# yoshitomo-matsubara/sc2-benchmark

Measured on AMD Instinct MI355X. Metric: images/s + bpp, Entropic-Student ResNet-50 224^2, higher is better.
Workload: dtype bf16

## Files before the change

include/sc2_bottleneck.h:

```cpp
#ifndef SC2_BOTTLENECK_H
#define SC2_BOTTLENECK_H

#include <stddef.h>
#include <stdint.h>

#ifdef __cplusplus
extern "C" {
#endif

#define SC2_OK 0
#define SC2_ERR_INVALID_ARG (-1)
#define SC2_ERR_UNSUPPORTED (-2)
#define SC2_ERR_DOMAIN (-3)
#define SC2_ERR_ZERO_PMF (-4)
#define SC2_ERR_LAUNCH (-5)
#define SC2_ERR_NO_DEVICE (-6)
#define SC2_ERR_INTERNAL (-7)

#define SC2_ABI_VERSION 51
int sc2_abi_version(void);

typedef struct sc2_policy {
    int32_t struct_bytes;
    int32_t conv_patch3;
// ... 81 lines not shown
    int32_t OH, OW;
    int32_t a_op;
    int32_t epilogue;
    int32_t out_format;
    int32_t Kpad;
    int32_t Cout_pad;
    int32_t out_H, out_W, out_stride_h, out_stride_w, out_off_h, out_off_w;
    int32_t k_order;
    int32_t dil_h, dil_w;
} sc2_conv_desc;

int sc2_conv_weight_rows(int Cout);
int sc2_conv_weight_pitch(int K);

int sc2_conv_fused_gdn_supported(const sc2_conv_desc *d);
int sc2_conv_patch_supported(const sc2_conv_desc *d);
int sc2_conv2d_fwd(const sc2_conv_desc *d, const void *x, const void *w_packed, void *y,
                   const void *ep_x, const float *ep_beta, void *stream);

int sc2_gdn1_bwd_gemm(const sc2_conv_desc *d, const void *x, const void *w_packed, void *y, void *y2, const void *ep_x,
                      const void *ep_x2, const float *ep_beta, void *stream);

int sc2_gdn1_rows_supported(int C);
int sc2_gdn1_rows_fwd(const void *x, const void *gamma_frag, const float *beta, void *y, long long M, int C, int inverse,
                      void *stream);
int sc2_gdn1_rows_bwd(const void *x, const void *gy, const void *gamma_frag, const void *gamma_t_frag, const float *beta,
                      void *d_norm, void *dx, float *d_beta, long long M, int C, int inverse, void *stream);
int sc2_colsum_bf16(const void *x, long long M, int C, float *out, void *stream);

int sc2_conv1x1_pair_supported(int K1, int C, int N2);
int sc2_conv1x1_pair_fwd(const void *o, const void *w3_frag, const float *b3, const void *identity, void *h,
                         const void *w1_frag, const float *b1, void *u, long long M, int K1, int C, int N2, void *stream);

int sc2_nchw_f32_to_nhwc_f32(const float *x, float *y, int N, int C, int H, int W, int Cpad, void *stream);
int sc2_conv_f32_chunk_channels(int Cout);
int sc2_conv2d_f32_fwd(const sc2_conv_desc *d, const float *x, const float *w_frag, void *y, const float *ep_x,
                       const float *ep_beta, void *stream);

int sc2_conv2x2_gdn512_supported(int Cin, int Cout, int KH, int KW, int stride, int pad);
int sc2_conv2x2_gdn512_fwd(const void *x, const void *w_packed, int Kpad, const void *gamma_frag, const float *beta,
                           void *y, void *t_out, int N, int H, int W, int Cin, int inverse, void *stream);

int sc2_conv0_gdn96_supported(int Cin_pairs, int Cout, int W_pairs);
int sc2_conv0_gdn96_fwd(const void *x_pairs, const void *w_frag, const void *gamma_frag, const float *beta, void *y, void *t_out,
                        int N, int H, int W_pairs, int inverse, void *stream);
int sc2_conv0_gdn96_nchw_fwd(const float *x_nchw, const void *w_frag, const void *gamma_frag, const float *beta, void *y,
                             int N, int H, int W, int inverse, void *stream);

int sc2_conv1x1_kres_supported(int Cin, int Cout, int stride);
int sc2_conv1x1_kres_fwd(const void *x, const void *w_frag, const float *bias, void *y, int N, int H, int W, int Cin, int Cout,
                         int stride, int relu, void *stream);

int sc2_conv2x2_c48_supported(int H, int W, int Cin, int Cout);
int sc2_conv2x2_c48_fwd(const void *x, const void *w_frag, const float *medians, void *y, int N, int H, int W, int Cin, int Cout,
                        int symbols, void *stream);

int sc2_conv1x1_win_supported(int Cin, int Cout, int stride);
int sc2_conv1x1_win_fwd(const void *x, const void *w_frag, const float *bias, const void *residual, const void *mask, void *y, int N,
                        int H, int W, int Cin, int Cout, int stride, int relu, void *stream);

int sc2_conv3x3_win_supported(int H, int W, int Cin, int Cout);
int sc2_conv3x3_win_fwd(const void *x, const void *w_frag, const float *bias, const void *mask, void *y, int N, int H, int W, int Cin,
                        int Cout, int relu, void *stream);

int sc2_conv3x3s2_win_supported(int H, int W, int Cin, int Cout);
int sc2_conv3x3s2_win_fwd(const void *x, const void *w_frag, const float *bias, void *y, int N, int H, int W, int Cin, int Cout,
// ... 133 lines not shown
```

sc2-benchmark_amd/build.py:

```python
import os
import subprocess
import sys
from concurrent.futures import ThreadPoolExecutor

HERE = os.path.dirname(os.path.abspath(__file__))
CSRC = os.path.join(HERE, 'csrc')
OBJ = os.path.join(CSRC, '_obj')
LIB = os.path.join(HERE, 'libsc2amd.so')
SOURCES = ['conv_inst_e.hip', 'conv_inst_f.hip', 'conv_inst_g.hip', 'conv_inst_h.hip', 'conv_inst_a.hip', 'conv_inst_b.hip',
           'conv_inst_c.hip', 'conv_inst_d.hip', 'conv_dec_persist.hip', 'conv_igemm.hip', 'conv_gdn512.hip', 'gdn512_rows.hip', 'bn.hip', 'gdn96_strips.hip', 'conv0_gdn96.hip', 'conv2_gdn48.hip', 'conv2x2_c48.hip', 'conv1x1_stream.hip', 'conv1x1_pair.hip', 'conv1x1_kres.hip', 'conv3x3_win.hip', 'conv1x1_win.hip', 'conv2x2_win.hip',
           'conv_f32.hip', 'loss.hip', 'conv_wgrad.hip', 'gdn_bwd.hip', 'entropy.hip', 'gaussian.hip', 'ar_context.hip', 'rans.hip', 'layout.hip', 'diag.hip', 'abi.cpp', 'cdf_host.cpp', 'rans_host.cpp']
HEADERS = [os.path.join(CSRC, 'sc2_common.h'), os.path.join(CSRC, 'conv_igemm_impl.h'),
           os.path.join(HERE, '..', 'include', 'sc2_bottleneck.h')]
HIPCC = os.environ.get('HIPCC', '/opt/rocm/bin/hipcc')
FLAGS = ['--offload-arch=gfx950', '-O3', '-fPIC', '-std=c++17', '-Wall', '-Wno-unused-function',
         '-D__HIP_PLATFORM_AMD__=1']


def _stale(target, deps):
    if not os.path.exists(target):
        return True
    t = os.path.getmtime(target)
    return any(os.path.getmtime(d) > t for d in deps)


def _compile(src):
    path = os.path.join(CSRC, src)
    obj = os.path.join(OBJ, src + '.o')
    if _stale(obj, [path] + HEADERS):
        cmd = [HIPCC] + FLAGS + ['-x', 'hip', '-c', path, '-o', obj]
        subprocess.check_call(cmd)
    return obj


def build(force=False, verbose=False):
    os.makedirs(OBJ, exist_ok=True)
    if force:
        for f in os.listdir(OBJ):
            os.remove(os.path.join(OBJ, f))
    with ThreadPoolExecutor(max_workers=min(8, os.cpu_count() or 1)) as ex:
        objs = list(ex.map(_compile, SOURCES))
    if _stale(LIB, objs):
        cmd = [HIPCC, '--offload-arch=gfx950', '-shared', '-fPIC', '-o', LIB] + objs
# ... 9 lines not shown
```

sc2-benchmark_amd/head.py:

```python
import os

import torch
from torch import nn

from . import hip
from .resnet import Bottleneck, FrozenBatchNorm2d


def _fold(conv, bn):
    w = conv.weight.detach().float()
    if bn is None:
        scale = torch.ones(w.shape[0], dtype=torch.float32, device=w.device)
        bias = torch.zeros(w.shape[0], dtype=torch.float32, device=w.device)
    elif isinstance(bn, (nn.BatchNorm2d, FrozenBatchNorm2d)):
        gamma = bn.weight.detach().float() if bn.weight is not None else torch.ones_like(bn.running_mean)
        beta = bn.bias.detach().float() if bn.bias is not None else torch.zeros_like(bn.running_mean)
        scale = gamma * torch.rsqrt(bn.running_var.detach().float() + bn.eps)
        bias = beta - bn.running_mean.detach().float() * scale
    else:
        raise TypeError('cannot fold {}'.format(type(bn)))
    w = w * scale.reshape(-1, 1, 1, 1)
    order = hip.preferred_k_order(w.shape[1], w.shape[2], w.shape[3])
    return hip.pack_conv_weight(w, order), bias.contiguous(), order, w

# ... 86 lines not shown
        if self.w_win1 is not None and epilogue in (hip.EPI_BIAS, hip.EPI_BIAS_RELU, hip.EPI_BIAS_ADD_RELU) and \
                max(x.numel(), x.shape[0] * x.shape[1] * x.shape[2] * self.cout) * 2 < 0x7FF00000:
            return hip.conv1x1_win_fwd(x, self.w_win1, self.b, stride=self.stride[0],
                                       residual=ep_x if epilogue == hip.EPI_BIAS_ADD_RELU else None,
                                       relu=epilogue != hip.EPI_BIAS, tag=self.tag)
        if self.stream and epilogue in (hip.EPI_BIAS, hip.EPI_BIAS_RELU, hip.EPI_BIAS_ADD_RELU):
            return hip.conv1x1_stream_fwd(x, self.w_frag, self.b, stride=self.stride[0],
                                          residual=ep_x if epilogue == hip.EPI_BIAS_ADD_RELU else None,
                                          relu=epilogue != hip.EPI_BIAS, tag=self.tag)
        if self.kres and epilogue in (hip.EPI_BIAS, hip.EPI_BIAS_RELU):
            return hip.conv1x1_kres_fwd(x, self.w_frag, self.b, stride=self.stride[0], relu=epilogue == hip.EPI_BIAS_RELU,
                                        tag=self.tag)
        if self.w_win is not None and epilogue in (hip.EPI_BIAS, hip.EPI_BIAS_RELU) and x.numel() * 2 < 0x7FF00000 and \
                hip.conv3x3_win_supported(x.shape[1], x.shape[2], x.shape[3], self.cout, self.k[0], self.k[1], self.stride, self.pad):
            return hip.conv3x3_win_fwd(x, self.w_win, self.b, relu=epilogue == hip.EPI_BIAS_RELU, tag=self.tag, stride=self.stride[0])
        return hip.conv2d_fwd(x, self.w, self.cout, self.k[0], self.k[1], self.stride, self.pad, epilogue=epilogue,
                              ep_x=ep_x, ep_beta=self.b, tag=self.tag, k_order=self.k_order)


class HipHead(object):

    def __init__(self, layers, fc):
        self.blocks = []
        for li, layer in layers:
            for bi, blk in enumerate(layer):
                if not isinstance(blk, Bottleneck):
                    raise hip.Sc2Error('HipHead supports torchvision Bottleneck blocks, got {}'.format(type(blk)))
                t = 'head.{}.{}'.format(li, bi)
                ds = None
                if blk.downsample is not None:
                    ds = _Conv(blk.downsample[0], blk.downsample[1], t + '.ds')
                self.blocks.append((_Conv(blk.conv1, blk.bn1, t + '.c1'), _Conv(blk.conv2, blk.bn2, t + '.c2'),
                                    _Conv(blk.conv3, blk.bn3, t + '.c3'), ds))
        self.fc = None
        if fc is not None:
            w = fc.weight.detach().float().reshape(fc.out_features, fc.in_features, 1, 1)
            cout_pad = (fc.out_features + 7) // 8 * 8
            if cout_pad != fc.out_features:
                w = torch.cat([w, torch.zeros(cout_pad - fc.out_features, fc.in_features, 1, 1, device=w.device)])
            b = torch.zeros(cout_pad, device=w.device)
            if fc.bias is not None:
                b[:fc.out_features] = fc.bias.detach().float()
            self.fc = (hip.pack_conv_weight(w), b.contiguous(), cout_pad, fc.out_features)
            self.fc_frag = None
            if fc.in_features % 128 == 0 and hip.host_policy.fc_kernel:
                n16 = (fc.out_features + 15) // 16 * 16
                w16 = torch.zeros(n16, fc.in_features, device=w.device)
                w16[:fc.out_features] = fc.weight.detach().float()
                b16 = torch.zeros(n16, device=w.device)
                if fc.bias is not None:
                    b16[:fc.out_features] = fc.bias.detach().float()
                self.fc_frag = (hip.pack_weight_fragments(w16), b16.contiguous())

    @staticmethod
    def _pair_ok(c3, c1n):
        return (c3.k == (1, 1) and c1n.k == (1, 1) and c3.stride == (1, 1) and c1n.stride == (1, 1) and c3.stream and
                c3.w2d is not None and c1n.w2d is not None and c3.w2d.shape[0] == c1n.w2d.shape[1] and
                hip.conv1x1_pair_supported(c3.w2d.shape[1], c3.cout, c1n.cout))

    @staticmethod
    def _pair_w1(c1n):
        if getattr(c1n, 'w_frag_pair', None) is None:
            c1n.w_frag_pair = hip.pack_weight_fragments(c1n.w_folded.reshape(c1n.w_folded.shape[0], c1n.w_folded.shape[1]))
        return c1n.w_frag_pair

    def tail_spec(self):
        c1, _, _, ds = self.blocks[0]
        if ds is None or c1.w2d is None or ds.w2d is None:
            return None
        if tuple(c1.w2d.shape) != (128, 256) or c1.stride != (1, 1) or tuple(ds.w2d.shape) != (512, 256) or ds.stride != (2, 2):
            return None
        return c1.w2d, c1.b, ds.w2d, ds.b

    def _side_stream(self, t):
        if not t.is_cuda or torch.cuda.is_current_stream_capturing():
            return None
        cur = torch.cuda.current_stream(t.device)
        pool = self.__dict__.setdefault('_side_streams', {})
        s = pool.get(cur.cuda_stream)
        if s is None:
            s = pool[cur.cuda_stream] = torch.cuda.Stream(device=t.device)
        return s

    def forward(self, x_nhwc, with_pool=True, pre=None):
        h = x_nhwc
        o_next = None
        side = self._side_stream(h if h is not None else pre[0]) if hip.host_policy.head_ds_side_stream else None
        for bi, (c1, c2, c3, ds) in enumerate(self.blocks):
            join = None
            if bi == 0 and pre is not None:
                o, identity = pre
            else:
                if ds is not None and side is not None:
                    cur = torch.cuda.current_stream(h.device)
                    fork = torch.cuda.Event()
                    fork.record(cur)
                    side.wait_event(fork)
                    h.record_stream(side)
                    with torch.cuda.stream(side):
                        identity = ds(h, hip.EPI_BIAS)
                        join = torch.cuda.Event()
                        join.record(side)
                    identity.record_stream(cur)
                else:
                    identity = h if ds is None else ds(h, hip.EPI_BIAS)
                o = o_next if o_next is not None else c1(h, hip.EPI_BIAS_RELU)
            o_next = None
            o = c2(o, hip.EPI_BIAS_RELU)
            if join is not None:
                torch.cuda.current_stream(h.device).wait_event(join)
            nxt = self.blocks[bi + 1] if bi + 1 < len(self.blocks) else None
            if nxt is not None and self._pair_ok(c3, nxt[0]) and o.numel() // o.shape[-1] * c3.cout * 2 < 0x7FF00000:
                h, o_next = hip.conv1x1_pair_fwd(o, c3.w_frag, c3.b, identity.contiguous(), self._pair_w1(nxt[0]), nxt[0].b,
                                                 tag=c3.tag + '+' + nxt[0].tag)
            else:
                h = c3(o, hip.EPI_BIAS_ADD_RELU, ep_x=identity)
        if not with_pool:
            return h.permute(0, 3, 1, 2)
        if self.fc is None:
            return hip.avgpool_nhwc(h.contiguous(), want_f32=True)[0]
        w, b, cout_pad, n_cls = self.fc
# ... 45 lines not shown
```

sc2-benchmark_amd/hip.py:

```python
import ctypes
import os

import torch

_HERE = os.path.dirname(os.path.abspath(__file__))
LIB_PATH = os.environ.get('SC2_LIB') or os.path.join(_HERE, 'libsc2amd.so')
_lib = None

AOP_NONE, AOP_ABS, AOP_SQUARE = 0, 1, 2
EPI_NONE, EPI_GDN, EPI_IGDN, EPI_BIAS, EPI_BIAS_RELU, EPI_BIAS_ADD_RELU, EPI_FUSED_GDN, EPI_FUSED_IGDN, \
    EPI_BIAS_LEAKY_RELU, EPI_GDN2, EPI_IGDN2 = range(11)
FUSABLE_GDN_CHANNELS = (32, 48, 64, 96)
OUT_BF16_NHWC, OUT_F32_NCHW, OUT_F32_NHWC, OUT_I32_NCHW_SYM = 0, 1, 2, 3
EB_NOISE, EB_DEQUANTIZE = 0, 1
EB_PARAM_STRIDE = 64

ABI_SYMBOLS = [
    'sc2_abi_version', 'sc2_last_error', 'sc2_device_count', 'sc2_policy_default', 'sc2_policy_set', 'sc2_policy_get',
    'sc2_nchw_f32_to_nhwc_bf16', 'sc2_nhwc_bf16_to_nchw_f32', 'sc2_avgpool_nhwc', 'sc2_maxpool_nhwc', 'sc2_bn_ws_floats', 'sc2_bn_train_fwd', 'sc2_bn_train_bwd', 'sc2_fc_fwd',
    'sc2_conv_weight_rows', 'sc2_conv_weight_pitch', 'sc2_conv_fused_gdn_supported', 'sc2_conv_patch_supported',
    'sc2_conv2d_fwd', 'sc2_gdn1_bwd_gemm', 'sc2_colsum_bf16', 'sc2_nchw_f32_to_nhwc_f32', 'sc2_conv_f32_chunk_channels', 'sc2_conv2d_f32_fwd',
    'sc2_conv2x2_gdn512_supported', 'sc2_conv2x2_gdn512_fwd', 'sc2_conv1x1_stream_supported', 'sc2_conv1x1_stream_mask_supported', 'sc2_conv1x1_stream_fwd', 'sc2_conv1x1_pair_supported', 'sc2_conv1x1_pair_fwd',
    'sc2_conv0_gdn96_supported', 'sc2_conv0_gdn96_fwd', 'sc2_conv0_gdn96_nchw_fwd', 'sc2_conv2_gdn48_supported', 'sc2_conv2_gdn48_fwd', 'sc2_conv2x2_c48_supported', 'sc2_conv2x2_c48_fwd', 'sc2_conv1x1_kres_supported', 'sc2_conv1x1_kres_fwd', 'sc2_conv1x1_win_supported', 'sc2_conv1x1_win_fwd', 'sc2_conv3x3_win_supported', 'sc2_conv3x3_win_fwd', 'sc2_conv3x3s2_win_supported', 'sc2_conv3x3s2_win_fwd', 'sc2_conv2x2_win_supported', 'sc2_conv2x2_win_fwd', 'sc2_conv2x2_win_tail_supported', 'sc2_conv2x2_win_tail_fwd', 'sc2_conv2d_wgrad', 'sc2_gdn_bwd_pre', 'sc2_gdn_bwd_post', 'sc2_gdn1_rows_supported', 'sc2_gdn1_rows_fwd', 'sc2_gdn1_rows_bwd',
    'sc2_eb_forward', 'sc2_eb_backward', 'sc2_eb_bits_partial_len', 'sc2_eb_symbols', 'sc2_eb_dequantize',
    'sc2_gc_forward', 'sc2_gc_backward', 'sc2_gc_symbols_indexes', 'sc2_gc_dequantize',
    'sc2_pmf_to_quantized_cdf',
    'sc2_rans_max_bytes', 'sc2_rans_workspace_bytes', 'sc2_rans_encode_batch', 'sc2_rans_decode_batch', 'sc2_rans_decode_dequantize_batch', 'sc2_rans_decode_dequantize_batch_ev',
    'sc2_mse_partial_len', 'sc2_mse_sum_bf16', 'sc2_mse_grad_bf16', 'sc2_relu_bwd_bf16', 'sc2_relu_bwd_mse_bf16',
    'sc2_ar_scan', 'sc2_rans_decode_resume',
    'sc2_rans_host_tables_create', 'sc2_rans_host_tables_destroy', 'sc2_rans_host_rcp_div', 'sc2_rans_code_host', 'sc2_clock_probe', 'sc2_rans_encode_host', 'sc2_rans_decode_host',
]


class ConvDesc(ctypes.Structure):
    _fields_ = [(n, ctypes.c_int32) for n in (
        'N', 'H', 'W', 'Cin', 'Cout', 'KH', 'KW', 'stride_h', 'stride_w', 'pad_h', 'pad_w', 'OH', 'OW',
        'a_op', 'epilogue', 'out_format', 'Kpad', 'Cout_pad', 'out_H', 'out_W', 'out_stride_h', 'out_stride_w',
        'out_off_h', 'out_off_w', 'k_order', 'dil_h', 'dil_w')]


class ArScanArgs(ctypes.Structure):
    _fields_ = ([(n, ctypes.c_int32) for n in ('B', 'H', 'W', 'M', 'C1p', 'C2p', 'n_table', 'n_cdfs', 'cdf_stride', 'pix0',
                                               'pix1', 'decode')] +
                [('scale_bound', ctypes.c_float), ('cdf_entries', ctypes.c_int32), ('stride', ctypes.c_int64)] +
                [(n, ctypes.c_void_p) for n in ('wc', 'bc', 'w1', 'p1', 'w2', 'b2', 'w3', 'b3', 'scale_table', 'y_hat_pad',
                                                'y_hat_nhwc', 'y', 'symbols', 'indexes', 'buf', 'io_offset', 'io_nbytes',
                                                'cdfs', 'cdf_sizes', 'offsets', 'st_x', 'st_pos', 'status',
                                                'gaussian_params')])


class Sc2Error(RuntimeError):
    pass


POLICY_FIELDS = ('struct_bytes', 'conv_patch3', 'conv_s2', 'conv_persist', 'conv_half', 'conv_big4', 'conv_no_big', 'conv_force_big',
                 'conv_no_epx', 'conv_debug', 'conv_chunk', 'w2_run', 'win_half', 'win_dbg', 'win_stamps', 'p1_half',
                 'p1_nbuf', 'pair_alt', 'f32_persist0', 'dec_stagger', 'wgrad_wgs', 'rans_lds_pad_kb', 'rans_pad_waves', 'rans_ragged2',
                 'rans_ragged2_waves', 'rans_lut8', 'rans_dq_lds', 'wgrad_ct')


class Policy(ctypes.Structure):
    _fields_ = [(n, ctypes.c_int32) for n in POLICY_FIELDS] + [('reserved', ctypes.c_int32 * 6)]


class HostPolicy(object):
    conv_patch = True
    k_order_tap = False
    b_tile_major = True
    conv0_fused = True
    conv2_fused = True
    conv_kres = 1
    conv_win = True
    conv_win_s2 = True
    conv2x2_win = True
    w2_tail = True
    conv_stream = True
    conv1x1_pair = True
    conv_c48 = True
    conv1x1_win = '1'
    conv_dilation = True
    fc_kernel = True
    dense_head = True
    rans_fused_dq = True
    gdn_rows = True
    gdn_bwd_fused = True
    dgrad_win_halves = True
    train_fused_conv2 = True
    train_fused_dec0 = True
    train_fused_conv0 = True
    bn_train_hip = True
    conv_train_hip = True
    pack_gather = True
    maxpool_hip = True
    relu_mask_fused = True
    mse_fused = True
    teacher_stream = True
    host_coder_max_streams = 64
    head_ds_side_stream = False
    pipeline_host_steps = True
    eval_graphs = True
    eval_graph_max_batch = 1


host_policy = HostPolicy()


def get_policy():
    p = Policy()
    lib().sc2_policy_get(ctypes.byref(p))
    return p
# ... 68 lines not shown
    L.sc2_conv_weight_rows.argtypes = [i32]
    L.sc2_conv_weight_pitch.argtypes = [i32]
    L.sc2_conv_fused_gdn_supported.argtypes = [ctypes.POINTER(ConvDesc)]
    L.sc2_conv_patch_supported.argtypes = [ctypes.POINTER(ConvDesc)]
    L.sc2_conv2d_fwd.argtypes = [ctypes.POINTER(ConvDesc), vp, vp, vp, vp, vp, vp]
    L.sc2_gdn1_bwd_gemm.argtypes = [ctypes.POINTER(ConvDesc), vp, vp, vp, vp, vp, vp, vp, vp]
    L.sc2_colsum_bf16.argtypes = [vp, ctypes.c_longlong, i32, vp, vp]
    L.sc2_nchw_f32_to_nhwc_f32.argtypes = [vp, vp, i32, i32, i32, i32, i32, vp]
    L.sc2_conv_f32_chunk_channels.argtypes = [i32]
    L.sc2_conv2d_f32_fwd.argtypes = [ctypes.POINTER(ConvDesc), vp, vp, vp, vp, vp, vp]
    L.sc2_conv2x2_gdn512_supported.argtypes = [i32] * 6
    L.sc2_conv2x2_gdn512_fwd.argtypes = [vp, vp, i32, vp, vp, vp, vp, i32, i32, i32, i32, i32, vp]
    L.sc2_conv0_gdn96_supported.argtypes = [i32, i32, i32]
    L.sc2_conv0_gdn96_fwd.argtypes = [vp, vp, vp, vp, vp, vp, i32, i32, i32, i32, vp]
    L.sc2_conv0_gdn96_nchw_fwd.argtypes = [vp, vp, vp, vp, vp, i32, i32, i32, i32, vp]
    L.sc2_conv1x1_kres_supported.argtypes = [i32, i32, i32]
    L.sc2_conv1x1_kres_fwd.argtypes = [vp, vp, vp, vp, i32, i32, i32, i32, i32, i32, i32, vp]
    L.sc2_conv3x3_win_supported.argtypes = [i32, i32, i32, i32]
    L.sc2_conv3x3_win_fwd.argtypes = [vp, vp, vp, vp, vp, i32, i32, i32, i32, i32, i32, vp]
    L.sc2_conv3x3s2_win_supported.argtypes = [i32, i32, i32, i32]
    L.sc2_conv1x1_win_supported.argtypes = [i32, i32, i32]
    L.sc2_conv2x2_c48_supported.argtypes = [i32, i32, i32, i32]
    L.sc2_conv2x2_c48_fwd.argtypes = [vp, vp, vp, vp, i32, i32, i32, i32, i32, i32, vp]
    L.sc2_conv1x1_win_fwd.argtypes = [vp, vp, vp, vp, vp, vp, i32, i32, i32, i32, i32, i32, i32, vp]
    L.sc2_conv3x3s2_win_fwd.argtypes = [vp, vp, vp, vp, i32, i32, i32, i32, i32, i32, vp]
    L.sc2_conv2x2_win_supported.argtypes = [i32, i32, i32, i32, i32]
    L.sc2_conv2x2_win_fwd.argtypes = [vp, vp, vp, vp, i32, i32, i32, i32, i32, i32, i32, i32, i32, vp]
    L.sc2_conv2x2_win_tail_supported.argtypes = [i32, i32, i32]
    L.sc2_conv2x2_win_tail_fwd.argtypes = [vp, vp, vp, vp, vp, vp, vp, i32, i32, i32, i32, vp]
    L.sc2_conv2_gdn48_supported.argtypes = [i32, i32, i32]
    L.sc2_conv2_gdn48_fwd.argtypes = [vp, vp, vp, vp, vp, vp, i32, i32, i32, i32, vp]
    L.sc2_conv1x1_pair_supported.argtypes = [i32, i32, i32]
    L.sc2_conv1x1_pair_fwd.argtypes = [vp, vp, vp, vp, vp, vp, vp, vp, ctypes.c_longlong, i32, i32, i32, vp]
    L.sc2_conv1x1_stream_supported.argtypes = [i32, i32, i32]
    L.sc2_conv1x1_stream_fwd.argtypes = [vp, vp, vp, vp, vp, vp, i32, i32, i32, i32, i32, i32, i32, vp]
    L.sc2_conv1x1_stream_mask_supported.argtypes = [i32, i32, i32]
    L.sc2_conv2d_wgrad.argtypes = [ctypes.POINTER(ConvDesc), vp, vp, vp, vp]
    L.sc2_gdn1_rows_supported.argtypes = [i32]
    L.sc2_gdn1_rows_fwd.argtypes = [vp, vp, vp, vp, ctypes.c_longlong, i32, i32, vp]
    L.sc2_gdn1_rows_bwd.argtypes = [vp, vp, vp, vp, vp, vp, vp, vp, ctypes.c_longlong, i32, i32, vp]
    L.sc2_gdn_bwd_pre.argtypes = [vp, vp, vp, ctypes.c_longlong, i32, i32, vp, vp, vp, vp]
    L.sc2_gdn_bwd_post.argtypes = [vp, vp, vp, ctypes.c_longlong, vp, vp]
    L.sc2_eb_forward.argtypes = [vp, vp, vp, i32, i32, i32, i32, f32, vp, vp, vp, vp, i32, vp]
    L.sc2_eb_backward.argtypes = [vp, vp, vp, i32, i32, i32, i32, f32, vp, vp, vp, vp, i32, vp]
    L.sc2_eb_bits_partial_len.argtypes = [i32, i32, i32]
    L.sc2_gc_forward.argtypes = [vp, vp, i64, vp, i64, vp, i64, i64, i32, f32, f32, vp, vp, vp]
    L.sc2_gc_backward.argtypes = [vp, vp, i64, vp, i64, vp, i64, i64, f32, f32, vp, vp, vp, vp, vp, vp]
    L.sc2_gc_symbols_indexes.argtypes = [vp, vp, i64, vp, i64, i64, i64, vp, i32, f32, vp, vp, vp]
    L.sc2_gc_dequantize.argtypes = [vp, vp, i64, i64, i32, i32, vp, vp, vp]
    L.sc2_eb_symbols.argtypes = [vp, vp, i32, i32, i32, vp, vp]
    L.sc2_eb_dequantize.argtypes = [vp, vp, i32, i32, i32, vp, vp, vp]
    L.sc2_pmf_to_quantized_cdf.argtypes = [ctypes.POINTER(ctypes.c_float), i32, i32,
                                           ctypes.POINTER(ctypes.c_uint32)]
    L.sc2_rans_max_bytes.argtypes = [i64]
    L.sc2_rans_max_bytes.restype = i64
    L.sc2_rans_workspace_bytes.argtypes = [i32, i64, i32, i32]
    L.sc2_rans_workspace_bytes.restype = i64
    L.sc2_rans_encode_batch.argtypes = [vp, vp, i64, i32, i64, vp, i32, i32, vp, vp, vp, i64, vp, vp, vp, vp, i64, vp]
    L.sc2_rans_decode_batch.argtypes = [vp, i64, vp, vp, vp, i64, i32, i64, vp, i32, i32, vp, vp, vp, vp, vp, i64,
                                        vp]
    L.sc2_rans_decode_dequantize_batch.argtypes = [vp, i64, vp, vp, i64, i32, i64, vp, i32, i32, vp, vp, vp, vp, vp, vp, vp, i64, vp]
    L.sc2_rans_decode_dequantize_batch_ev.argtypes = [vp, i64, vp, vp, i64, i32, i64, vp, i32, i32, vp, vp, vp, vp, vp, vp, vp, i64, vp, vp, vp]
    L.sc2_mse_partial_len.argtypes = [ctypes.c_longlong]
    L.sc2_mse_sum_bf16.argtypes = [vp, vp, ctypes.c_longlong, vp, vp]
    L.sc2_mse_grad_bf16.argtypes = [vp, vp, ctypes.c_longlong, vp, vp, vp]
    L.sc2_relu_bwd_bf16.argtypes = [vp, vp, vp, ctypes.c_longlong, vp, vp]
# ... 789 lines not shown
    OH, OW = (H - 1) // stride + 1, (W - 1) // stride + 1
    out = torch.empty((N, OH, OW, cout), dtype=torch.bfloat16, device=x_nhwc.device)
    if residual is not None:
        _dev(residual, 'residual')
        assert residual.dtype == torch.bfloat16 and residual.is_contiguous() and tuple(residual.shape) == tuple(out.shape)
    if mask is not None:
        _dev(mask, 'mask')
        assert not relu and mask.dtype == torch.bfloat16 and mask.is_contiguous() and tuple(mask.shape) == tuple(out.shape)
    with _timed(tag or 'conv1x1_stream'):
        _check(lib().sc2_conv1x1_stream_fwd(_ptr(x_nhwc), _ptr(w_frag), _ptr(bias), _ptr(residual), _ptr(mask), _ptr(out), N, H, W,
                                            Cin, cout, int(stride), 1 if relu else 0, _stream()), 'conv1x1_stream_fwd')
    return out


def conv1x1_pair_supported(k1, c, n2):
    return host_policy.conv1x1_pair and bool(lib().sc2_conv1x1_pair_supported(k1, c, n2))


def conv1x1_pair_fwd(o_nhwc, w3_frag, b3, identity, w1_frag, b1, tag=None):
    for t, name in ((o_nhwc, 'o'), (w3_frag, 'w3_frag'), (b3, 'b3'), (identity, 'identity'), (w1_frag, 'w1_frag'), (b1, 'b1')):
        _dev(t, name)
        assert t.is_contiguous(), name
    N, H, W, K1 = o_nhwc.shape
    C, N2 = w3_frag.shape[0] * 16, w1_frag.shape[0] * 16
    assert o_nhwc.dtype == torch.bfloat16 and identity.dtype == torch.bfloat16 and tuple(identity.shape) == (N, H, W, C)
    assert tuple(w3_frag.shape) == (C // 16, K1 // 32, 64, 8) and tuple(w1_frag.shape) == (N2 // 16, C // 32, 64, 8)
    assert b3.dtype == torch.float32 and b3.numel() == C and b1.dtype == torch.float32 and b1.numel() == N2
    h = torch.empty((N, H, W, C), dtype=torch.bfloat16, device=o_nhwc.device)
    u = torch.empty((N, H, W, N2), dtype=torch.bfloat16, device=o_nhwc.device)
    with _timed(tag or 'conv1x1_pair'):
        _check(lib().sc2_conv1x1_pair_fwd(_ptr(o_nhwc), _ptr(w3_frag), _ptr(b3), _ptr(identity), _ptr(h), _ptr(w1_frag), _ptr(b1),
                                          _ptr(u), N * H * W, K1, C, N2, _stream()), 'conv1x1_pair_fwd')
    return h, u


def conv2x2_c48_supported(x_shape, cout, kh, kw, stride, pad):
    sh, sw = (stride, stride) if isinstance(stride, int) else stride
    ph, pw = (pad, pad) if isinstance(pad, int) else pad
    if not host_policy.conv_c48:
        return False
    N, H, W, Cin = x_shape
    if N * H * W * Cin * 2 >= 0x7FF00000:
        return False
    return (kh, kw, sh, sw, ph, pw) == (2, 2, 1, 1, 0, 0) and bool(lib().sc2_conv2x2_c48_supported(H, W, Cin, cout))


def pack_conv2x2_c48(w):
    _dev(w, 'w')
    cout = w.shape[0]
    assert tuple(w.shape[1:]) == (48, 2, 2) and cout <= 32
    w2d = torch.zeros((32, 192), dtype=torch.float32, device=w.device)
    w2d[:cout] = w.detach().float().permute(0, 2, 3, 1).reshape(cout, 192)
    return pack_weight_fragments(w2d)


def conv2x2_c48_fwd(x_nhwc, w_frag, cout, medians=None, tag=None, out=None):
    for t, name in ((x_nhwc, 'x'), (w_frag, 'w_frag')):
        _dev(t, name)
    assert x_nhwc.dtype == torch.bfloat16 and x_nhwc.dim() == 4 and x_nhwc.is_contiguous()
    N, H, W, Cin = x_nhwc.shape
    assert w_frag.dtype == torch.bfloat16 and w_frag.is_contiguous() and tuple(w_frag.shape) == (2, 6, 64, 8)
    sym = medians is not None
    if sym:
        _dev(medians, 'medians')
        assert medians.dtype == torch.float32 and medians.is_contiguous() and medians.numel() == cout
    dt = torch.int32 if sym else torch.float32
# ... 627 lines not shown
```

Before: 36340.

## Fuse consecutive ResNet-50 layer3 identity bottlenecks into one persistent per-image kernel

Adds a HIP kernel that runs up to five consecutive 1024->256->256->1024 identity bottleneck blocks at 14x14 in one launch. Each workgroup holds a whole image: it streams the input through LDS slabs for conv1, keeps the mid activations in LDS for the 3x3 conv and conv3, then adds the residual and applies ReLU in place. The goal is to remove the intermediate HBM round trips and per-conv launch overhead. The cost is one workgroup per image, which relies on the batch filling the CUs (checked by the supported test), and weights are re-read from global memory by every workgroup.

```diff
diff --git a/include/sc2_bottleneck.h b/include/sc2_bottleneck.h
--- a/include/sc2_bottleneck.h
+++ b/include/sc2_bottleneck.h
@@ -137,6 +137,11 @@
 int sc2_conv1x1_pair_fwd(const void *o, const void *w3_frag, const float *b3, const void *identity, void *h,
                          const void *w1_frag, const float *b1, void *u, long long M, int K1, int C, int N2, void *stream);
 
+int sc2_conv1x1_block3_supported(int C, int mid, int H, int W, int N);
+int sc2_conv1x1_block3_fwd(const void *x, void *y, const void *const *w1_frag, const void *const *w2_frag, const void *const *w3_frag,
+                           const float *const *b1, const float *const *b2, const float *const *b3, int n_blocks, int N, int C,
+                           int mid, int H, int W, void *stream);
+
 int sc2_nchw_f32_to_nhwc_f32(const float *x, float *y, int N, int C, int H, int W, int Cpad, void *stream);
 int sc2_conv_f32_chunk_channels(int Cout);
 int sc2_conv2d_f32_fwd(const sc2_conv_desc *d, const float *x, const float *w_frag, void *y, const float *ep_x,
diff --git a/sc2-benchmark_amd/build.py b/sc2-benchmark_amd/build.py
--- a/sc2-benchmark_amd/build.py
+++ b/sc2-benchmark_amd/build.py
@@ -8,7 +8,7 @@
 OBJ = os.path.join(CSRC, '_obj')
 LIB = os.path.join(HERE, 'libsc2amd.so')
 SOURCES = ['conv_inst_e.hip', 'conv_inst_f.hip', 'conv_inst_g.hip', 'conv_inst_h.hip', 'conv_inst_a.hip', 'conv_inst_b.hip',
-           'conv_inst_c.hip', 'conv_inst_d.hip', 'conv_dec_persist.hip', 'conv_igemm.hip', 'conv_gdn512.hip', 'gdn512_rows.hip', 'bn.hip', 'gdn96_strips.hip', 'conv0_gdn96.hip', 'conv2_gdn48.hip', 'conv2x2_c48.hip', 'conv1x1_stream.hip', 'conv1x1_pair.hip', 'conv1x1_kres.hip', 'conv3x3_win.hip', 'conv1x1_win.hip', 'conv2x2_win.hip',
+           'conv_inst_c.hip', 'conv_inst_d.hip', 'conv_dec_persist.hip', 'conv_igemm.hip', 'conv_gdn512.hip', 'gdn512_rows.hip', 'bn.hip', 'gdn96_strips.hip', 'conv0_gdn96.hip', 'conv2_gdn48.hip', 'conv2x2_c48.hip', 'conv1x1_stream.hip', 'conv1x1_pair.hip', 'conv1x1_block3.hip', 'conv1x1_kres.hip', 'conv3x3_win.hip', 'conv1x1_win.hip', 'conv2x2_win.hip',
            'conv_f32.hip', 'loss.hip', 'conv_wgrad.hip', 'gdn_bwd.hip', 'entropy.hip', 'gaussian.hip', 'ar_context.hip', 'rans.hip', 'layout.hip', 'diag.hip', 'abi.cpp', 'cdf_host.cpp', 'rans_host.cpp']
 HEADERS = [os.path.join(CSRC, 'sc2_common.h'), os.path.join(CSRC, 'conv_igemm_impl.h'),
            os.path.join(HERE, '..', 'include', 'sc2_bottleneck.h')]
diff --git a/sc2-benchmark_amd/csrc/conv1x1_block3.hip b/sc2-benchmark_amd/csrc/conv1x1_block3.hip
--- /dev/null
+++ b/sc2-benchmark_amd/csrc/conv1x1_block3.hip
@@ -0,0 +1,314 @@
+#include <stdlib.h>
+
+#include "sc2_common.h"
+
+namespace {
+
+typedef float f32x2_t __attribute__((ext_vector_type(2)));
+typedef __bf16 bf16x2_t __attribute__((ext_vector_type(2)));
+__device__ __forceinline__ uint32_t pack2(f32x2_t v) {
+    return __builtin_bit_cast(uint32_t, __builtin_convertvector(v, bf16x2_t));
+}
+
+#if defined(__HIP_DEVICE_COMPILE__)
+typedef __amdgpu_buffer_rsrc_t buf_rsrc_t;
+__device__ __forceinline__ buf_rsrc_t make_rsrc(const void *base, uint32_t bytes) {
+    return __builtin_amdgcn_make_buffer_rsrc(const_cast<void *>(base), 0, (int)bytes, 0x00020000);
+}
+constexpr int kSc1 = 16;
+__device__ __forceinline__ uint4 buf_load16(buf_rsrc_t r, uint32_t voff, uint32_t soff) {
+    return __builtin_bit_cast(uint4, __builtin_amdgcn_raw_buffer_load_b128(r, (int)voff, (int)soff, 0));
+}
+__device__ __forceinline__ uint4 buf_load16_sc1(buf_rsrc_t r, uint32_t voff, uint32_t soff) {
+    return __builtin_bit_cast(uint4, __builtin_amdgcn_raw_buffer_load_b128(r, (int)voff, (int)soff, kSc1));
+}
+__device__ __forceinline__ void buf_store16(buf_rsrc_t r, uint32_t voff, uint32_t soff, uint4 v) {
+    __builtin_amdgcn_raw_buffer_store_b128(__builtin_bit_cast(__attribute__((ext_vector_type(4))) unsigned, v), r, (int)voff,
+                                           (int)soff, 0);
+    __builtin_amdgcn_sched_barrier(0);
+    asm volatile("s_nop 1" ::: "memory");
+    __builtin_amdgcn_sched_barrier(0);
+}
+#else
+typedef int buf_rsrc_t;
+__device__ __forceinline__ buf_rsrc_t make_rsrc(const void *, uint32_t) { return 0; }
+__device__ __forceinline__ uint4 buf_load16(buf_rsrc_t, uint32_t, uint32_t) { return make_uint4(0, 0, 0, 0); }
+__device__ __forceinline__ uint4 buf_load16_sc1(buf_rsrc_t, uint32_t, uint32_t) { return make_uint4(0, 0, 0, 0); }
+__device__ __forceinline__ void buf_store16(buf_rsrc_t, uint32_t, uint32_t, uint4) {}
+#endif
+
+constexpr int kMaxBlocks = 5;
+constexpr int HW = 14, NPIX = HW * HW;
+constexpr int PT = (NPIX + 15) / 16;
+constexpr int C = 1024, MID = 256;
+constexpr int RS = MID * 2 + 16;
+constexpr int ZROW = PT * 16;
+constexpr int IMG = (ZROW + 1) * RS;
+constexpr int SLAB_CH = 128, SROW = SLAB_CH * 2, SLAB = PT * 16 * SROW;
+constexpr int NSLAB = C / SLAB_CH;
+constexpr int BIAS_OFF = IMG;
+constexpr int LDS_BYTES = IMG + (MID + MID + C) * 4;
+constexpr int SQ = (NPIX * (SROW / 16) + 511) / 512;
+constexpr int SKS = SLAB_CH / 32;
+constexpr uint32_t OOB = 0x80000000u;
+static_assert(2 * SLAB <= ZROW * RS, "the slabs overlay the image but never its zero row");
+static_assert(IMG % 16 == 0 && LDS_BYTES <= 160 * 1024, "LDS budget");
+
+struct Block3Args {
+    const uint16_t *x;
+    uint16_t *y;
+    const uint16_t *w1[kMaxBlocks];
+    const uint16_t *w2[kMaxBlocks];
+    const uint16_t *w3[kMaxBlocks];
+    const float *b1[kMaxBlocks], *b2[kMaxBlocks], *b3[kMaxBlocks];
+    int n_img, n_blocks;
+};
+
+template <typename Addr>
+__device__ __forceinline__ void kstep(f32x4_t (&acc)[PT][2], const uint4 (&w)[2], Addr addr, const unsigned char *smem) {
+    const bf16x8_t w0 = __builtin_bit_cast(bf16x8_t, w[0]), w1 = __builtin_bit_cast(bf16x8_t, w[1]);
+#pragma unroll
+    for (int pt = 0; pt < PT; ++pt) {
+        const bf16x8_t xf = __builtin_bit_cast(bf16x8_t, *reinterpret_cast<const uint4 *>(smem + addr(pt)));
+        acc[pt][0] = __builtin_amdgcn_mfma_f32_16x16x32_bf16(w0, xf, acc[pt][0], 0, 0, 0);
+        acc[pt][1] = __builtin_amdgcn_mfma_f32_16x16x32_bf16(w1, xf, acc[pt][1], 0, 0, 0);
+    }
+    __builtin_amdgcn_sched_barrier(0);
+}
+
+__device__ __forceinline__ void zero_acc(f32x4_t (&acc)[PT][2]) {
+#pragma unroll
+    for (int pt = 0; pt < PT; ++pt) acc[pt][0] = acc[pt][1] = f32x4_t{0.f, 0.f, 0.f, 0.f};
+}
+
+__device__ __forceinline__ void store_image(const f32x4_t (&acc)[PT][2], const float *bias, unsigned char *smem, int wn, int frow,
+                                            int fq) {
+#pragma unroll
+    for (int j = 0; j < 2; ++j) {
+        const int ch = (2 * wn + j) * 16 + fq * 4;
+        const float4 bv = *reinterpret_cast<const float4 *>(bias + ch);
+        const f32x2_t b01 = {bv.x, bv.y}, b23 = {bv.z, bv.w};
+#pragma unroll
+        for (int pt = 0; pt < PT; ++pt) {
+            f32x2_t v01 = f32x2_t{acc[pt][j][0], acc[pt][j][1]} + b01;
+            f32x2_t v23 = f32x2_t{acc[pt][j][2], acc[pt][j][3]} + b23;
+            v01 = f32x2_t{fmaxf(v01[0], 0.f), fmaxf(v01[1], 0.f)};
+            v23 = f32x2_t{fmaxf(v23[0], 0.f), fmaxf(v23[1], 0.f)};
+            uint2 o;
+            o.x = pack2(v01);
+            o.y = pack2(v23);
+            *reinterpret_cast<uint2 *>(smem + (pt * 16 + frow) * RS + ch * 2) = o;
+        }
+    }
+}
+
+__global__ __launch_bounds__(512, 1) void conv1x1_block3_kernel(const Block3Args p) {
+    extern __shared__ __attribute__((aligned(16))) unsigned char smem[];
+    float *bias = reinterpret_cast<float *>(smem + BIAS_OFF);
+
+    const int tid = threadIdx.x, lane = tid & 63;
+    const int wn = __builtin_amdgcn_readfirstlane(tid >> 6);
+    const int frow = lane & 15, fq = lane >> 4;
+    const int img = blockIdx.x;
+    const uint32_t img_off = (uint32_t)img * (NPIX * C * 2);
+
+    const buf_rsrc_t rs_x = make_rsrc(p.x, (uint32_t)p.n_img * (NPIX * C * 2));
+    const buf_rsrc_t rs_y = make_rsrc(p.y, (uint32_t)p.n_img * (NPIX * C * 2));
+    const uint32_t w_vo = (uint32_t)lane * 16u;
+
+    for (int k = tid; k < RS / 16; k += 512) *reinterpret_cast<uint4 *>(smem + ZROW * RS + k * 16) = make_uint4(0, 0, 0, 0);
+
+    f32x4_t acc[PT][2];
+#pragma unroll 1
+    for (int blk = 0; blk < p.n_blocks; ++blk) {
+        const buf_rsrc_t rs_in = blk == 0 ? rs_x : rs_y;
+        const buf_rsrc_t rs_w1 = make_rsrc(p.w1[blk], MID * C * 2);
+        const buf_rsrc_t rs_w2 = make_rsrc(p.w2[blk], MID * MID * 9 * 2);
+        const buf_rsrc_t rs_w3 = make_rsrc(p.w3[blk], C * MID * 2);
+
+        uint4 sv[SQ];
+        auto load_slab = [&](int s) {
+#pragma unroll
+            for (int k = 0; k < SQ; ++k) {
+                const int q = tid + 512 * k;
+                const bool ok = q < NPIX * (SROW / 16);
+                sv[k] = buf_load16_sc1(rs_in, ok ? (uint32_t)((q >> 4) * (C * 2) + (q & 15) * 16) : OOB, img_off + s * SROW);
+            }
+        };
+        auto store_slab = [&](int buf) {
+#pragma unroll
+            for (int k = 0; k < SQ; ++k) {
+                const int q = tid + 512 * k;
+                if (q < NPIX * (SROW / 16))
+                    *reinterpret_cast<uint4 *>(smem + buf * SLAB + (q >> 4) * SROW + (((q & 15) ^ ((q >> 4) & 15)) << 4)) = sv[k];
+            }
+        };
+        load_slab(0);
+        static_assert(MID + MID + C == 3 * 512, "three bias words per thread");
+        bias[tid] = tid < MID ? p.b1[blk][tid] : p.b2[blk][tid - MID];
+        bias[512 + tid] = p.b3[blk][tid];
+        bias[1024 + tid] = p.b3[blk][512 + tid];
+        store_slab(0);
+        load_slab(1);
+        uint4 wb[2][2];
+        {
+            constexpr int KS = C / 32;
+#pragma unroll
+            for (int g = 0; g < 2; ++g)
+#pragma unroll
+                for (int j = 0; j < 2; ++j) wb[g][j] = buf_load16(rs_w1, w_vo, (uint32_t)(((2 * wn + j) * KS + g) * 1024));
+            const uint32_t sa0 = (uint32_t)(frow * SROW + ((fq ^ frow) << 4));
+            zero_acc(acc);
+            __syncthreads();
+#pragma unroll 1
+            for (int s = 0; s < NSLAB; ++s) {
+                const uint32_t base = (uint32_t)((s & 1) * SLAB);
+#pragma unroll
+                for (int ks = 0; ks < SKS; ++ks) {
+                    const int g = SKS * s + ks, h = ks & 1;
+                    uint4 w[2] = {wb[h][0], wb[h][1]};
+                    const int gn = g + 2 < KS ? g + 2 : KS - 1;
+#pragma unroll
+                    for (int j = 0; j < 2; ++j) wb[h][j] = buf_load16(rs_w1, w_vo, (uint32_t)(((2 * wn + j) * KS + gn) * 1024));
+                    const uint32_t sa = base + (sa0 ^ (uint32_t)(ks << 6));
+                    kstep(acc, w, [&](int pt) { return sa + pt * (16 * SROW); }, smem);
+                }
+                if (s + 1 < NSLAB) store_slab((s + 1) & 1);
+                if (s + 2 < NSLAB) load_slab(s + 2);
+                __syncthreads();
+            }
+        }
+        store_image(acc, bias, smem, wn, frow, fq);
+        {
+            constexpr int KS = 9 * MID / 32, KT = MID / 32;
+#pragma unroll
+            for (int g = 0; g < 2; ++g)
+#pragma unroll
+                for (int j = 0; j < 2; ++j) wb[g][j] = buf_load16(rs_w2, w_vo, (uint32_t)(((2 * wn + j) * KS + g) * 1024));
+            zero_acc(acc);
+            __syncthreads();
+#pragma unroll 1
+            for (int tap = 0; tap < 9; ++tap) {
+                const int dy = tap / 3 - 1, dx = tap % 3 - 1;
+                int lr = frow;
+                asm volatile("" : "+v"(lr));
+                uint32_t a[PT];
+#pragma unroll
+                for (int pt = 0; pt < PT; ++pt) {
+                    const int q = pt * 16 + lr;
+                    const int y = q / HW, x = q - (q / HW) * HW;
+                    const bool ok = q < NPIX && (unsigned)(y + dy) < (unsigned)HW && (unsigned)(x + dx) < (unsigned)HW;
+                    a[pt] = (uint32_t)((ok ? q + dy * HW + dx : ZROW) * RS + fq * 16);
+                }
+#pragma unroll
+                for (int ks = 0; ks < KT; ++ks) {
+                    const int g = tap * KT + ks, h = ks & 1;
+                    uint4 w[2] = {wb[h][0], wb[h][1]};
+                    const int gn = g + 2 < KS ? g + 2 : KS - 1;
+#pragma unroll
+                    for (int j = 0; j < 2; ++j) wb[h][j] = buf_load16(rs_w2, w_vo, (uint32_t)(((2 * wn + j) * KS + gn) * 1024));
+                    kstep(acc, w, [&](int pt) { return a[pt] + ks * 64; }, smem);
+                }
+            }
+        }
+        __syncthreads();
+        store_image(acc, bias + MID, smem, wn, frow, fq);
+        {
+            constexpr int KS = MID / 32;
+            const uint32_t a0 = (uint32_t)(frow * RS + fq * 16);
+            __syncthreads();
+#pragma unroll 1
+            for (int n = 0; n < C / MID; ++n) {
+                const int jt0 = n * (MID / 16) + 2 * wn;
+#pragma unroll
+                for (int g = 0; g < 2; ++g)
+#pragma unroll
+                    for (int j = 0; j < 2; ++j) wb[g][j] = buf_load16(rs_w3, w_vo, (uint32_t)(((jt0 + j) * KS + g) * 1024));
+                zero_acc(acc);
+#pragma unroll
+                for (int ks = 0; ks < KS; ++ks) {
+                    const int h = ks & 1;
+                    uint4 w[2] = {wb[h][0], wb[h][1]};
+                    if (ks + 2 < KS) {
+#pragma unroll
+                        for (int j = 0; j < 2; ++j) wb[h][j] = buf_load16(rs_w3, w_vo, (uint32_t)(((jt0 + j) * KS + ks + 2) * 1024));
+                    }
+                    kstep(acc, w, [&](int pt) { return a0 + pt * (16 * RS) + ks * 64; }, smem);
+                }
+                {
+                    const int ch = n * MID + wn * 32 + fq * 8;
+                    const float4 ba = *reinterpret_cast<const float4 *>(bias + 2 * MID + ch);
+                    const float4 bb = *reinterpret_cast<const float4 *>(bias + 2 * MID + ch + 4);
+                    const f32x2_t bv[4] = {{ba.x, ba.y}, {ba.z, ba.w}, {bb.x, bb.y}, {bb.z, bb.w}};
+                    uint4 r[PT];
+#pragma unroll
+                    for (int pt = 0; pt < PT; ++pt) {
+                        const int q = pt * 16 + frow;
+                        r[pt] = buf_load16_sc1(rs_in, q < NPIX ? (uint32_t)(q * (C * 2) + ch * 2) : OOB, img_off);
+                    }
+#pragma unroll
+                    for (int pt = 0; pt < PT; ++pt) {
+                        const int q = pt * 16 + frow;
+                        const uint32_t rw[4] = {r[pt].x, r[pt].y, r[pt].z, r[pt].w};
+                        uint32_t o[4];
+#pragma unroll
+                        for (int e = 0; e < 4; ++e) {
+                            const f32x4_t &a = acc[pt][e >> 1];
+                            f32x2_t v = f32x2_t{a[(e & 1) * 2], a[(e & 1) * 2 + 1]} + bv[e];
+                            v += f32x2_t{__builtin_bit_cast(float, rw[e] << 16), __builtin_bit_cast(float, rw[e] & 0xFFFF0000u)};
+                            o[e] = pack2(f32x2_t{fmaxf(v[0], 0.f), fmaxf(v[1], 0.f)});
+                        }
+                        buf_store16(rs_y, q < NPIX ? (uint32_t)(q * (C * 2) + ch * 2) : OOB, img_off, make_uint4(o[0], o[1], o[2], o[3]));
+                    }
+                }
+            }
+        }
+        asm volatile("s_waitcnt vmcnt(0)" ::: "memory");
+        __syncthreads();
+    }
+}
+
+}
+
+extern "C" int sc2_conv1x1_block3_supported(int C_, int mid, int H, int W, int N) {
+    if (C_ != C || mid != MID || H != HW || W != HW || N < 1) return 0;
+    const int cus = sc2_device_cus();
+    const long long rounds = (N + cus - 1) / cus;
+    return 4LL * N >= 3LL * rounds * cus ? 1 : 0;
+}
+
+extern "C" int sc2_conv1x1_block3_fwd(const void *x, void *y, const void *const *w1_frag, const void *const *w2_frag,
+                                      const void *const *w3_frag, const float *const *b1, const float *const *b2,
+                                      const float *const *b3, int n_blocks, int N, int C_, int mid, int H, int W, void *stream) {
+    SC2_REQUIRE(x && y && w1_frag && w2_frag && w3_frag && b1 && b2 && b3, SC2_ERR_INVALID_ARG, "conv1x1_block3: null argument");
+    SC2_REQUIRE(C_ == C && mid == MID && H == HW && W == HW, SC2_ERR_UNSUPPORTED,
+                "conv1x1_block3: C %d mid %d %d x %d not supported", C_, mid, H, W);
+    SC2_REQUIRE(n_blocks >= 1 && n_blocks <= kMaxBlocks, SC2_ERR_INVALID_ARG, "conv1x1_block3: %d blocks (1..%d)", n_blocks, kMaxBlocks);
+    SC2_REQUIRE(N >= 1 && (long long)N * NPIX * C * 2 < 0x7FF00000LL, SC2_ERR_UNSUPPORTED,
+                "conv1x1_block3: N = %d outside the 32-bit buffer range", N);
+    SC2_REQUIRE(x != y, SC2_ERR_INVALID_ARG, "conv1x1_block3: x and y must not alias");
+    Block3Args a;
+    a.x = static_cast<const uint16_t *>(x);
+    a.y = static_cast<uint16_t *>(y);
+    for (int b = 0; b < kMaxBlocks; ++b) {
+        const int s = b < n_blocks ? b : 0;
+        SC2_REQUIRE(w1_frag[s] && w2_frag[s] && w3_frag[s] && b1[s] && b2[s] && b3[s], SC2_ERR_INVALID_ARG,
+                    "conv1x1_block3: null weight of block %d", s);
+        a.w1[b] = static_cast<const uint16_t *>(w1_frag[s]);
+        a.w2[b] = static_cast<const uint16_t *>(w2_frag[s]);
+        a.w3[b] = static_cast<const uint16_t *>(w3_frag[s]);
+        a.b1[b] = b1[s]; a.b2[b] = b2[s]; a.b3[b] = b3[s];
+    }
+    a.n_img = N;
+    a.n_blocks = n_blocks;
+    static bool attr_set[SC2_MAX_DEVICES] = {};
+    const int dev = sc2_device_slot();
+    if (!attr_set[dev]) {
+        (void)hipFuncSetAttribute(reinterpret_cast<const void *>(&conv1x1_block3_kernel), hipFuncAttributeMaxDynamicSharedMemorySize,
+                                  LDS_BYTES);
+        attr_set[dev] = true;
+    }
+    hipLaunchKernelGGL(conv1x1_block3_kernel, dim3(N), dim3(512), LDS_BYTES, static_cast<hipStream_t>(stream), a);
+    SC2_CHECK_LAUNCH();
+    return SC2_OK;
+}
diff --git a/sc2-benchmark_amd/head.py b/sc2-benchmark_amd/head.py
--- a/sc2-benchmark_amd/head.py
+++ b/sc2-benchmark_amd/head.py
@@ -142,6 +142,7 @@
                     ds = _Conv(blk.downsample[0], blk.downsample[1], t + '.ds')
                 self.blocks.append((_Conv(blk.conv1, blk.bn1, t + '.c1'), _Conv(blk.conv2, blk.bn2, t + '.c2'),
                                     _Conv(blk.conv3, blk.bn3, t + '.c3'), ds))
+        self.block3 = [self._block3_pack(*b) for b in self.blocks]
         self.fc = None
         if fc is not None:
             w = fc.weight.detach().float().reshape(fc.out_features, fc.in_features, 1, 1)
@@ -163,6 +164,28 @@
                 self.fc_frag = (hip.pack_weight_fragments(w16), b16.contiguous())
 
     @staticmethod
+    def _block3_pack(c1, c2, c3, ds):
+        identity_block = (ds is None and c1.k == (1, 1) and c3.k == (1, 1) and c2.k == (3, 3) and c1.stride == (1, 1) and
+                          c2.stride == (1, 1) and c3.stride == (1, 1) and c2.pad == (1, 1) and
+                          c1.dilation == c2.dilation == c3.dilation == (1, 1))
+        w1, w2, w3 = c1.w_folded, c2.w_folded, c3.w_folded
+        if not identity_block or tuple(w1.shape) != (256, 1024, 1, 1) or tuple(w2.shape) != (256, 256, 3, 3) or \
+                tuple(w3.shape) != (1024, 256, 1, 1):
+            return None
+        return hip.pack_block3_weights(w1, w2, w3), c1.b, c2.b, c3.b
+
+    def _block3_run(self, bi, h):
+        if h is None or h.dim() != 4 or self.block3[bi] is None:
+            return 0
+        N, H, W, C = h.shape
+        if not hip.conv1x1_block3_supported(C, 256, H, W, N) or N * H * W * C * 2 >= 0x7FF00000:
+            return 0
+        n = 1
+        while n < 5 and bi + n < len(self.blocks) and self.block3[bi + n] is not None:
+            n += 1
+        return n
+
+    @staticmethod
     def _pair_ok(c3, c1n):
         return (c3.k == (1, 1) and c1n.k == (1, 1) and c3.stride == (1, 1) and c1n.stride == (1, 1) and c3.stream and
                 c3.w2d is not None and c1n.w2d is not None and c3.w2d.shape[0] == c1n.w2d.shape[1] and
@@ -196,7 +219,17 @@
         h = x_nhwc
         o_next = None
         side = self._side_stream(h if h is not None else pre[0]) if hip.host_policy.head_ds_side_stream else None
+        skip = 0
         for bi, (c1, c2, c3, ds) in enumerate(self.blocks):
+            if skip:
+                skip -= 1
+                continue
+            run = self._block3_run(bi, h) if o_next is None and not (bi == 0 and pre is not None) else 0
+            if run:
+                h = hip.conv1x1_block3_fwd(h.contiguous(), self.block3[bi:bi + run],
+                                           tag=c1.tag[:-3] + ('-' + self.blocks[bi + run - 1][0].tag[5:-3] if run > 1 else ''))
+                skip = run - 1
+                continue
             join = None
             if bi == 0 and pre is not None:
                 o, identity = pre
diff --git a/sc2-benchmark_amd/hip.py b/sc2-benchmark_amd/hip.py
--- a/sc2-benchmark_amd/hip.py
+++ b/sc2-benchmark_amd/hip.py
@@ -20,7 +20,7 @@
     'sc2_nchw_f32_to_nhwc_bf16', 'sc2_nhwc_bf16_to_nchw_f32', 'sc2_avgpool_nhwc', 'sc2_maxpool_nhwc', 'sc2_bn_ws_floats', 'sc2_bn_train_fwd', 'sc2_bn_train_bwd', 'sc2_fc_fwd',
     'sc2_conv_weight_rows', 'sc2_conv_weight_pitch', 'sc2_conv_fused_gdn_supported', 'sc2_conv_patch_supported',
     'sc2_conv2d_fwd', 'sc2_gdn1_bwd_gemm', 'sc2_colsum_bf16', 'sc2_nchw_f32_to_nhwc_f32', 'sc2_conv_f32_chunk_channels', 'sc2_conv2d_f32_fwd',
-    'sc2_conv2x2_gdn512_supported', 'sc2_conv2x2_gdn512_fwd', 'sc2_conv1x1_stream_supported', 'sc2_conv1x1_stream_mask_supported', 'sc2_conv1x1_stream_fwd', 'sc2_conv1x1_pair_supported', 'sc2_conv1x1_pair_fwd',
+    'sc2_conv2x2_gdn512_supported', 'sc2_conv2x2_gdn512_fwd', 'sc2_conv1x1_stream_supported', 'sc2_conv1x1_stream_mask_supported', 'sc2_conv1x1_stream_fwd', 'sc2_conv1x1_pair_supported', 'sc2_conv1x1_pair_fwd', 'sc2_conv1x1_block3_supported', 'sc2_conv1x1_block3_fwd',
     'sc2_conv0_gdn96_supported', 'sc2_conv0_gdn96_fwd', 'sc2_conv0_gdn96_nchw_fwd', 'sc2_conv2_gdn48_supported', 'sc2_conv2_gdn48_fwd', 'sc2_conv2x2_c48_supported', 'sc2_conv2x2_c48_fwd', 'sc2_conv1x1_kres_supported', 'sc2_conv1x1_kres_fwd', 'sc2_conv1x1_win_supported', 'sc2_conv1x1_win_fwd', 'sc2_conv3x3_win_supported', 'sc2_conv3x3_win_fwd', 'sc2_conv3x3s2_win_supported', 'sc2_conv3x3s2_win_fwd', 'sc2_conv2x2_win_supported', 'sc2_conv2x2_win_fwd', 'sc2_conv2x2_win_tail_supported', 'sc2_conv2x2_win_tail_fwd', 'sc2_conv2d_wgrad', 'sc2_gdn_bwd_pre', 'sc2_gdn_bwd_post', 'sc2_gdn1_rows_supported', 'sc2_gdn1_rows_fwd', 'sc2_gdn1_rows_bwd',
     'sc2_eb_forward', 'sc2_eb_backward', 'sc2_eb_bits_partial_len', 'sc2_eb_symbols', 'sc2_eb_dequantize',
     'sc2_gc_forward', 'sc2_gc_backward', 'sc2_gc_symbols_indexes', 'sc2_gc_dequantize',
@@ -76,6 +76,7 @@
     w2_tail = True
     conv_stream = True
     conv1x1_pair = True
+    head_block3 = True
     conv_c48 = True
     conv1x1_win = '1'
     conv_dilation = True
@@ -210,6 +211,8 @@
     L.sc2_conv2_gdn48_fwd.argtypes = [vp, vp, vp, vp, vp, vp, i32, i32, i32, i32, vp]
     L.sc2_conv1x1_pair_supported.argtypes = [i32, i32, i32]
     L.sc2_conv1x1_pair_fwd.argtypes = [vp, vp, vp, vp, vp, vp, vp, vp, ctypes.c_longlong, i32, i32, i32, vp]
+    L.sc2_conv1x1_block3_supported.argtypes = [i32, i32, i32, i32, i32]
+    L.sc2_conv1x1_block3_fwd.argtypes = [vp, vp, vp, vp, vp, vp, vp, vp, i32, i32, i32, i32, i32, i32, vp]
     L.sc2_conv1x1_stream_supported.argtypes = [i32, i32, i32]
     L.sc2_conv1x1_stream_fwd.argtypes = [vp, vp, vp, vp, vp, vp, i32, i32, i32, i32, i32, i32, i32, vp]
     L.sc2_conv1x1_stream_mask_supported.argtypes = [i32, i32, i32]
@@ -1065,6 +1068,40 @@
         _check(lib().sc2_conv1x1_pair_fwd(_ptr(o_nhwc), _ptr(w3_frag), _ptr(b3), _ptr(identity), _ptr(h), _ptr(w1_frag), _ptr(b1),
                                           _ptr(u), N * H * W, K1, C, N2, _stream()), 'conv1x1_pair_fwd')
     return h, u
+
+
+def conv1x1_block3_supported(c, mid, h, w, n):
+    return host_policy.head_block3 and bool(lib().sc2_conv1x1_block3_supported(c, mid, h, w, n))
+
+
+def pack_block3_weights(w1, w2, w3):
+    mid, c = w1.shape[0], w1.shape[1]
+    assert tuple(w2.shape) == (mid, mid, 3, 3) and tuple(w3.shape) == (c, mid, 1, 1) and c % 32 == 0
+    w3p = w3.reshape(c // 32, 4, 2, 4, mid).permute(0, 2, 1, 3, 4).reshape(c, mid)
+    return (pack_weight_fragments(w1.reshape(mid, c)), pack_weight_fragments(w2.permute(0, 2, 3, 1).reshape(mid, 9 * mid)),
+            pack_weight_fragments(w3p))
+
+
+def conv1x1_block3_fwd(x_nhwc, blocks, tag=None):
+    _dev(x_nhwc, 'x')
+    assert x_nhwc.dtype == torch.bfloat16 and x_nhwc.dim() == 4 and x_nhwc.is_contiguous()
+    assert 1 <= len(blocks) <= 5
+    N, H, W, C = x_nhwc.shape
+    arr = [(ctypes.c_void_p * 5)() for _ in range(6)]
+    for bi, ((w1, w2, w3), b1, b2, b3) in enumerate(blocks):
+        mid = w1.shape[0] * 16
+        assert tuple(w1.shape) == (mid // 16, C // 32, 64, 8) and tuple(w2.shape) == (mid // 16, 9 * mid // 32, 64, 8)
+        assert tuple(w3.shape) == (C // 16, mid // 32, 64, 8)
+        assert b1.numel() == mid and b2.numel() == mid and b3.numel() == C
+        for k, t in enumerate((w1, w2, w3, b1, b2, b3)):
+            _dev(t, 'block weight')
+            assert t.is_contiguous() and t.dtype == (torch.bfloat16 if k < 3 else torch.float32)
+            arr[k][bi] = t.data_ptr()
+    y = torch.empty_like(x_nhwc)
+    with _timed(tag or 'conv1x1_block3'):
+        _check(lib().sc2_conv1x1_block3_fwd(_ptr(x_nhwc), _ptr(y), *arr, len(blocks), N, C, mid, H, W, _stream()),
+               'conv1x1_block3_fwd')
+    return y
 
 
 def conv2x2_c48_supported(x_shape, cout, kh, kw, stride, pad):
```

Result: faster. 37380, median of 6 (+2.9%).
